# mathwrx/Decouple-and-Couple_Learning_in_Multi-Modal_Brain_Tumor_Segmentation

Hardware: AMD Instinct MI355X
Metric: training volumes/sec (4x128^3) (higher is better)
Workload: dtype bf16x3 forward (split-bf16 MFMA operands hi.hi+hi.lo+lo.hi: logits within 1e-3 of the fp32 reference) / bf16 data-gradient / bf16 weight-gradient MFMA operands; f32 accumulate, f32 storage, f32 master weights; 1 GPU; configs[1]: 1xMI355X, batch 2 per GPU, 4-modality 128^3 synthetic BraTS patches; fwd + softmax_dice + 4 sub-region/edge losses + bwd + Adam(amsgrad); random-init weights, dropout on; global_batch=2, parallelism=dp1, precision=bf16x3, dgrad_precision=bf16, wgrad_precision=bf16, mode=plan

## Files before the change

decouple-and-couple_learning_in_multi-modal_brain_tumor_segmentation_amd/csrc/wgrad_bf16.hip:

```cpp
#include "conv_args.h"
#include <type_traits>
#include <cstdlib>

typedef __bf16 bf16x8 __attribute__((ext_vector_type(8)));
typedef short s16x4 __attribute__((ext_vector_type(4)));
typedef __attribute__((address_space(3))) s16x4 lds_s16x4;

extern "C" int cwf_wgrad_nsplit(int op, int N, int Do, int Ho, int Wo, int Cin, int Cout);
constexpr int SIDE_WGS = 160;

struct WgArgsB {
  ConvGeom g;
  const float* x; const float* in_scale; const float* in_shift; float in_slope;
  const float* dy; int dy_ldc; float* partial;
  int ngroups, tiles_per_split, total_tiles;
  int64_t slab_floats;
  int cls_slab_base[8];
  int groups;
  const float* x_g[3]; const float* dy_g[3]; float* partial_g[3];
  const float* dy_scale;
};

__device__ __forceinline__ unsigned pack_bf16w(float a, float b) {
  const __bf16 x = (__bf16)a, y = (__bf16)b;
// ... 1031 lines not shown
#pragma unroll
    for (int i = 0; i < 7; ++i)
#pragma unroll
      for (int j = 0; j < NTW; ++j) acc[i][j] = (f32x4){0.f, 0.f, 0.f, 0.f};
    typedef short s16x8 __attribute__((ext_vector_type(8)));
    const s16x8 ones_s = {0x3F80, 0x3F80, 0x3F80, 0x3F80, 0x3F80, 0x3F80, 0x3F80, 0x3F80};
    const bf16x8 ones = __builtin_bit_cast(bf16x8, ones_s);
    const bool bias_wave = wave == 3;
    const unsigned lane_x = lds_base + (((kq & 1) * XW + (kq >> 1) * 8 + bq) * 16 + bp * 4) * 2;
    unsigned xa0[7];
#pragma unroll
    for (int i = 0; i < 7; ++i) {
      const int t = wave + 4 * i;
      xa0[i] = lane_x + (t < 27 ? (((t / 9) * 6 + (t / 3) % 3) * XW + t % 3) * 32 : 0);
    }
    const unsigned da0 = lds_base + WS1D_XIB + (((kq & 1) * DP + (kq >> 1) * 8 + bq) * CGW + (kq & 1) * DSK + bp * 4) * 2;
    auto trf = [&](unsigned addr, unsigned second) __attribute__((always_inline)) {
      const s16x4 u = __builtin_amdgcn_ds_read_tr16_b64_v4i16((lds_s16x4*)(uintptr_t)addr);
      const s16x4 v = __builtin_amdgcn_ds_read_tr16_b64_v4i16((lds_s16x4*)(uintptr_t)(addr + second));
      const s16x8 w = {u[0], u[1], u[2], u[3], v[0], v[1], v[2], v[3]};
      return __builtin_bit_cast(bf16x8, w);
    };
    for (int it = 0; it < niter; ++it) {
      asm volatile("s_barrier" ::: "memory");
      const unsigned bo = (unsigned)(it & 3) * WS1D_BUFB;
      unsigned xa[7];
#pragma unroll
      for (int i = 0; i < 7; ++i) xa[i] = xa0[i] + bo;
      const unsigned da = da0 + bo;
      constexpr int DEPTH = CWF_WS1_DEPTH;
      bf16x8 ah[DEPTH + 1], bh[2][NTW];
      auto issue = [&](int f) __attribute__((always_inline)) {
        const int ks = f / 7, i = f % 7;
        if (i == 0) {
          const unsigned od_ = (2 * ks * DP * CGW + ks * DSK) * 2;
#pragma unroll
          for (int j = 0; j < NTW; ++j) bh[ks & 1][j] = trf(da + od_ + j * 32, 4 * CGW * 2);
        }
        const unsigned ox = (((ks >> 1) * 6 + ((2 * ks) & 3)) * XW) * 32;
        ah[f % (DEPTH + 1)] = trf(xa[i] + ox, 4 * 32);
      };
#pragma unroll
      for (int f = 0; f < DEPTH; ++f) issue(f);
#pragma unroll
      for (int f = 0; f < 56; ++f) {
        if (f + DEPTH < 56) issue(f + DEPTH);
        __builtin_amdgcn_sched_barrier(0);
        const int ks = f / 7, i = f % 7;
        bf16x8 ahf = ah[f % (DEPTH + 1)];
        if (i == 6) ahf = bias_wave ? ones : ahf;
#pragma unroll
        for (int j = 0; j < NTW; ++j)
          acc[i][j] = __builtin_amdgcn_mfma_f32_16x16x32_bf16(ahf, bh[ks & 1][j], acc[i][j], 0, 0, 0);
        __builtin_amdgcn_sched_barrier(0);
      }
    }
    float4* out = reinterpret_cast<float4*>(a.partial + (int64_t)split * a.slab_floats);
#pragma unroll
    for (int i = 0; i < 7; ++i) {
      const int t = wave + 4 * i;
      if (t > 27) continue;
#pragma unroll
      for (int j = 0; j < NTW; ++j) {
        const int64_t blk = (((int64_t)chunk * a.ngroups + grp) * 28 + t) * CG + j;
        out[blk * 64 + lane] = make_float4(acc[i][j][0], acc[i][j][1], acc[i][j][2], acc[i][j][3]);
      }
    }
  } else {
    const int lw = wave - 4;
    typedef __attribute__((address_space(3))) void* lds_vp;
    typedef __attribute__((address_space(1))) const void* glb_vp;
    const int gx = a.Cin >> 3, gd = a.Cout >> 3;
    auto run = [&](auto NI_) __attribute__((always_inline)) {
      constexpr int NI = decltype(NI_)::value;
      int off[NI]; unsigned crd[NI];
#pragma unroll
      for (int k = 0; k < NI; ++k) {
        const int s = lw + WS1_LW * k;
        if (s < WS1D_XP) {
          const int gi = 64 * s + lane;
          const int row = gi / 40, gr = gi % 40, w = gr >> 1, half = gr & 1;
          const int c0 = row / 6, c1 = row % 6;
          off[k] = ((c0 * a.H + c1) * a.W + w) * gx + chunk * 2 + half;
          crd[k] = (unsigned)c0 | ((unsigned)c1 << 3) | ((unsigned)w << 6) | ((row < 36 && gr < 36) ? 1u << 11 : 0u);
        } else {
          const int m = s - WS1D_XP, w = lane >> 2, q = lane & 3;
          off[k] = (((m >> 2) * a.H + (m & 3)) * a.W + w) * gd + grp * 4 + q;
          crd[k] = (unsigned)(m >> 2) | ((unsigned)(m & 3) << 3) | ((unsigned)w << 6) | (1u << 11);
        }
      }
      auto issue = [&](int it) __attribute__((always_inline)) {
        const int tile = t_begin + it;
        const int n = tile / tiles_sp; int rem = tile - n * tiles_sp;
        const int tile_w = rem % a.tiles_w; rem /= a.tiles_w;
        const int tile_h = rem % a.tiles_h; const int tile_d = rem / a.tiles_h;
        const int od0 = tile_d * 4, oh0 = tile_h * 4, ow0 = tile_w * 16;
        const int64_t vd = (((int64_t)n * a.D + od0) * a.H + oh0) * a.W + ow0;
        const int64_t vx = vd - ((int64_t)a.H + 1) * a.W - 1;
        const unsigned lbuf = lds_base + (unsigned)(it & 3) * WS1D_BUFB;
#pragma unroll
        for (int k = 0; k < NI; ++k) {
          const int s = lw + WS1_LW * k;
          const bool isd = s >= WS1D_XP;
          const int c0 = (int)(crd[k] & 7u), c1 = (int)((crd[k] >> 3) & 7u), w = (int)((crd[k] >> 6) & 31u);
          const int gdd = (isd ? od0 : od0 - 1) + c0, gh = (isd ? oh0 : oh0 - 1) + c1, gw = (isd ? ow0 : ow0 - 1) + w;
          const bool ok = (crd[k] >> 11) != 0u && (unsigned)gdd < (unsigned)a.D && (unsigned)gh < (unsigned)a.H && (unsigned)gw < (unsigned)a.W;
          const uint4* src = (isd ? a.dy + vd * gd : a.xa + vx * gx) + off[k];
          src = ok ? src : a.zero;
          const int m = s - WS1D_XP;
          const unsigned dst = isd ? (unsigned)(WS1D_XIB + m * 1024 + ((m + 1) >> 1) * 32) : (unsigned)s * 1024u;
          __builtin_amdgcn_global_load_lds((glb_vp)src, (lds_vp)(uintptr_t)(lbuf + dst), 16, 0, 0);
        }
      };
      if (niter > 0) issue(0);
      if (niter > 1) issue(1);
      if (niter > 2) issue(2);
      for (int it = 0; it < niter; ++it) {
        if (it + 2 < niter) asm volatile("s_waitcnt vmcnt(%0)" :: "n"(2 * NI) : "memory");
        else asm volatile("s_waitcnt vmcnt(0)" ::: "memory");
        asm volatile("s_barrier" ::: "memory");
        if (it + 3 < niter) issue(it + 3);
      }
    };
    constexpr int NP = WS1D_XP + WS1D_DP;
    if (lw < NP % WS1_LW) run(std::integral_constant<int, NP / WS1_LW + 1>{});
    else run(std::integral_constant<int, NP / WS1_LW>{});
  }
}

static int wgrad_s1d_launch(const cwf_wgrad_args& d, int* nsplit_used, hipStream_t st) {
  const void* xa16 = d.xa16; const void* dy16 = d.dy16; const void* zero16 = d.zero16; float* partial = d.partial;
  const int N = d.N, D = d.Di, H = d.Hi, W = d.Wi, Cin = d.Cin, Cout = d.Cout;
  if (!xa16 || !dy16 || !zero16 || !partial || N <= 0 || D <= 0 || H <= 0 || W <= 0) return CWF_E_BADARG;
  if (((uintptr_t)xa16 & 15) || ((uintptr_t)dy16 & 15) || ((uintptr_t)zero16 & 15) || ((uintptr_t)partial & 15)) return CWF_E_ALIGN;
  if (Cin < 16 || (Cin & 15) || Cout < 32 || (Cout & 31)) return CWF_E_BADARG;
  if ((int64_t)N * D * H * W * (Cin > Cout ? Cin : Cout) >= (1ll << 33)) return CWF_E_TOOLARGE;
  Ws1dArgs a;
  a.xa = (const uint4*)xa16; a.dy = (const uint4*)dy16; a.zero = (const uint4*)zero16; a.partial = partial;
  a.N = N; a.D = D; a.H = H; a.W = W; a.Cin = Cin; a.Cout = Cout;
  a.tiles_d = cdiv(D, 4); a.tiles_h = cdiv(H, 4); a.tiles_w = cdiv(W, 16);
  a.total_tiles = N * a.tiles_d * a.tiles_h * a.tiles_w;
  const int nchunks = Cin / 16;
  a.ngroups = Cout / 32;
  const int nblk = nchunks * a.ngroups;
  a.slab_floats = (int64_t)nblk * 28 * 2 * 256;
  if (a.slab_floats != cwf_wgrad_slab_floats(CWF_CONV3_S1, Cin, Cout)) return CWF_E_BADARG;
  int want = SIDE_WGS / nblk; if (want < 1) want = 1; if (want > a.total_tiles) want = a.total_tiles;
  a.tiles_per_split = cdiv(a.total_tiles, want);
  const int splits = cdiv(a.total_tiles, a.tiles_per_split);
  if (splits > cwf_wgrad_nsplit(CWF_CONV3_S1, N, D, H, W, Cin, Cout)) return CWF_E_BADARG;
  const size_t lds = (size_t)WS1D_NBUF * WS1D_BUFB;
  CWF_MAX_LDS_ONCE((&wgrad_s1d_kernel));
  hipLaunchKernelGGL(wgrad_s1d_kernel, dim3(splits, nblk), dim3(256 + 64 * WS1_LW), lds, st, a);
  CWF_LAUNCH_CHECK();
  if (nsplit_used) *nsplit_used = splits;
  return 0;
}

struct PwWgWork { int Vin, gps, wps, gpw; };

template <int NCH, int NTL, int NCLS> struct PwgCfg { static constexpr int WAVES = (NCLS * NTL * (NCH + 1) <= 12) ? 16 : 8; };
template <int NCH, int NTL, int NCLS>
__global__ __launch_bounds__((64 * PwgCfg<NCH, NTL, NCLS>::WAVES)) void pw_wgrad_kernel(const WgArgsB a, const PwWgWork wk, int CG) {
  constexpr int PWG_WAVES = PwgCfg<NCH, NTL, NCLS>::WAVES, RB = 32 / PWG_WAVES;
  constexpr int G = (NCLS > 1) ? (NCH * NTL > 1 ? 1 : 2) : (NCH + NTL <= 2 ? 16 : (NCH + NTL <= 3 ? 12 : (NCH + NTL <= 6 ? 4 : 2)));
  __shared__ float4 red[PWG_WAVES][RB][64];
  const ConvGeom& g = a.g;
  const int tid = threadIdx.x, lane = tid & 63, li = lane & 15, lk = lane >> 4;
  const int wave = __builtin_amdgcn_readfirstlane(tid >> 6);
  const int n = (int)blockIdx.x / wk.wps, wg = (int)blockIdx.x % wk.wps;
  const int gA = (wg * PWG_WAVES + wave) * wk.gpw;
  const int gB = min(gA + wk.gpw, wk.gps);
  const float* xs = a.x + (int64_t)n * wk.Vin * g.x_ldc;
  const float* ds = a.dy + (int64_t)n * g.Do * g.Ho * g.Wo * a.dy_ldc;
  const bool has_norm = a.in_scale != nullptr;
  const bool plain = !has_norm && a.in_slope == 1.f;
  float sc[NCH], sh[NCH];
#pragma unroll
  for (int c = 0; c < NCH; ++c) {
    const int ci = c * 16 + li;
    sc[c] = (has_norm && ci < g.Cin) ? a.in_scale[(int64_t)n * g.Cin + ci] : 1.f;
    sh[c] = (has_norm && ci < g.Cin) ? a.in_shift[(int64_t)n * g.Cin + ci] : 0.f;
  }
  f32x4 acc[NCLS][NCH][NTL], accb[NCLS][NTL];
#pragma unroll
  for (int q = 0; q < NCLS; ++q)
#pragma unroll
    for (int t = 0; t < NTL; ++t) {
      accb[q][t] = (f32x4){0.f, 0.f, 0.f, 0.f};
#pragma unroll
      for (int c = 0; c < NCH; ++c) acc[q][c][t] = (f32x4){0.f, 0.f, 0.f, 0.f};
    }

  for (int gi = gA; gi < gB; gi += G) {
    float xv[G][NCH], dv[G][NCLS][NTL];
#pragma unroll
    for (int k = 0; k < G; ++k) {
      const bool ok = gi + k < gB;
      const int vox = (gi + k) * 4 + lk;
#pragma unroll
      for (int c = 0; c < NCH; ++c) {
        const int ci = c * 16 + li;
        xv[k][c] = (ok && ci < g.Cin) ? xs[(int64_t)vox * g.x_ldc + ci] : 0.f;
      }
      int64_t ov[NCLS];
      if (NCLS == 1) ov[0] = vox;
      else {
        const int w_ = vox % g.Wi, t2 = vox / g.Wi, h_ = t2 % g.Hi, d_ = t2 / g.Hi;
#pragma unroll
        for (int q = 0; q < NCLS; ++q) ov[q < NCLS ? q : 0] = ((int64_t)(2 * d_ + (q >> 2)) * g.Ho + 2 * h_ + ((q >> 1) & 1)) * g.Wo + 2 * w_ + (q & 1);
      }
#pragma unroll
      for (int q = 0; q < NCLS; ++q)
#pragma unroll
        for (int t = 0; t < NTL; ++t) {
          const int co = t * 16 + li;
          dv[k][q][t] = (ok && co < g.Cout) ? ds[ov[q] * a.dy_ldc + co] : 0.f;
        }
    }
#pragma unroll
    for (int k = 0; k < G; ++k) {
      const bool ok = gi + k < gB;
      float xa[NCH];
#pragma unroll
      for (int c = 0; c < NCH; ++c) {
        float v = xv[k][c];
        if (!plain) v = cwf_act(v * sc[c] + sh[c], a.in_slope);
        xa[c] = (ok && c * 16 + li < g.Cin) ? v : 0.f;
      }
#pragma unroll
      for (int q = 0; q < NCLS; ++q)
#pragma unroll
        for (int t = 0; t < NTL; ++t) {
          accb[q][t] = __builtin_amdgcn_mfma_f32_16x16x4f32(1.f, dv[k][q][t], accb[q][t], 0, 0, 0);
#pragma unroll
          for (int c = 0; c < NCH; ++c) acc[q][c][t] = __builtin_amdgcn_mfma_f32_16x16x4f32(xa[c], dv[k][q][t], acc[q][c][t], 0, 0, 0);
        }
    }
  }

  float4* out = reinterpret_cast<float4*>(a.partial + (int64_t)blockIdx.x * a.slab_floats);
  constexpr int NB = NCLS * NTL * (NCH + 1);
  f32x4 flat[NB]; int bid[NB];
  {
    int u = 0;
#pragma unroll
    for (int q = 0; q < NCLS; ++q)
#pragma unroll
      for (int t = 0; t < NTL; ++t) {
        const int grp = t / CG, j = t % CG;
#pragma unroll
        for (int c = 0; c < NCH; ++c) { flat[u] = acc[q][c][t]; bid[u] = a.cls_slab_base[q] + ((c * a.ngroups + grp) * 2) * CG + j; ++u; }
        flat[u] = accb[q][t]; bid[u] = a.cls_slab_base[q] + ((0 * a.ngroups + grp) * 2 + 1) * CG + j; ++u;
      }
  }
#pragma unroll
  for (int b0 = 0; b0 < NB; b0 += RB) {
    __syncthreads();
#pragma unroll
    for (int r_ = 0; r_ < RB; ++r_)
      if (b0 + r_ < NB) red[wave][r_][lane] = make_float4(flat[b0 + r_][0], flat[b0 + r_][1], flat[b0 + r_][2], flat[b0 + r_][3]);
    __syncthreads();
    if (wave < RB && b0 + wave < NB) {
      float4 sum = red[0][wave][lane];
#pragma unroll
      for (int w = 1; w < PWG_WAVES; ++w) { const float4 p = red[w][wave][lane]; sum.x += p.x; sum.y += p.y; sum.z += p.z; sum.w += p.w; }
      int id = bid[b0];
#pragma unroll
      for (int r_ = 1; r_ < RB; ++r_) if (b0 + r_ < NB && wave == r_) id = bid[b0 + r_];
      out[(int64_t)id * 64 + lane] = sum;
      if (NCH > 1) {
#pragma unroll
        for (int r_ = 0; r_ < RB; ++r_) {
          if (b0 + r_ < NB && wave == r_ && (b0 + r_) % (NCH + 1) == NCH) {
            for (int c = 1; c < NCH; ++c) out[((int64_t)id + (int64_t)c * a.ngroups * 2 * CG) * 64 + lane] = sum;
          }
        }
      }
    }
  }
}

template <int NCH, int NTL, int NCLS>
static int launch_pw_wgrad(const WgArgsB& a, int CG, int max_slabs, int* nsplit_used, hipStream_t st) {
  const ConvGeom& g = a.g;
  PwWgWork wk;
  wk.Vin = g.Di * g.Hi * g.Wi;
  wk.gps = wk.Vin >> 2;
  int wps = SIDE_WGS / g.N; if (wps < 1) wps = 1;
  if (wps * g.N > max_slabs) wps = max_slabs / g.N;
  if (wps < 1) return -1;
  constexpr int PWG_WAVES = PwgCfg<NCH, NTL, NCLS>::WAVES;
  const int maxw = cdiv(wk.gps, PWG_WAVES * 8);
  if (wps > maxw) wps = maxw;
  wk.gpw = cdiv(wk.gps, wps * PWG_WAVES);
  wk.wps = cdiv(wk.gps, wk.gpw * PWG_WAVES);
  hipLaunchKernelGGL((pw_wgrad_kernel<NCH, NTL, NCLS>), dim3((unsigned)(wk.wps * g.N)), dim3(64 * PWG_WAVES), 0, st, a, wk, CG);
  CWF_LAUNCH_CHECK();
  if (nsplit_used) *nsplit_used = wk.wps * g.N;
  return 0;
}

static int wgrad_bf16_impl(const cwf_wgrad_args& d, int* nsplit_used, hipStream_t st) {
  const int op = d.op, x3 = d.precision == CWF_BF16X3, groups = d.groups, N = d.N, Cin = d.Cin, Cout = d.Cout;
  const int Di = d.Di, Hi = d.Hi, Wi = d.Wi, Do = d.Do, Ho = d.Ho, Wo = d.Wo, x_ldc = d.x_ldc, dy_ldc = d.dy_ldc;
  const float* x = groups ? d.x_g[0] : d.x; const float* dy = groups ? d.dy_g[0] : d.dy; float* partial = groups ? d.partial_g[0] : d.partial;
  const float* in_scale = d.in_scale; const float* dy_scale = d.dy_scale;
  if (!x || !dy || !partial || N <= 0) return CWF_E_BADARG;
  if (dy_scale && !(!groups && op == CWF_CONV3_S1 && Cin <= 16 && Cout == 16 && (dy_ldc & 3) == 0 && (((uintptr_t)dy) & 15) == 0 && (int64_t)Do * Ho * Wo >= 32768))
    return CWF_E_BADARG;
  if ((Cin & 3) || (x_ldc & 3) || ((uintptr_t)x & 15) || ((uintptr_t)partial & 15)) return CWF_E_ALIGN;
  if (in_scale && !d.in_shift) return CWF_E_BADARG;
  if (!(op == CWF_CONV3_S1 || op == CWF_CONV3_S2 || op == CWF_CONV1 || op == CWF_CONVT2)) return CWF_E_BADARG;
  const bool tapsplit = (op == CWF_CONV3_S1 || op == CWF_CONV3_S2);
  const int MTOT = (op == CWF_CONV3_S2) ? 4 : 16;
  const int nt_all = cdiv(Cout, 16);
  const int CG = tapsplit ? (nt_all == 1 ? 1 : 2) : (nt_all == 1 ? 1 : (nt_all == 2 ? 2 : 4));
  WgArgsB a;
  int rc = cwf_build_geom(a.g, op, N, Di, Hi, Wi, Cin, x_ldc, Do, Ho, Wo, Cout, dy_ldc, MTOT);
  if (rc) return rc;
  const int nchunks = a.g.nchunks, ncls = a.g.ncls, ngroups = cdiv(a.g.ntiles, CG);
  int64_t blocks = 0;
  for (int c = 0; c < 8; ++c) { a.cls_slab_base[c] = (int)blocks; if (c < ncls) blocks += (int64_t)nchunks * ngroups * (a.g.cls_ntaps[c] + 1) * CG; }
  const int total = N * a.g.tiles_d * a.g.tiles_h * a.g.tiles_w;
  const int nblk = nchunks * ngroups * ncls;
  int want = 512 / nblk; if (want < 1) want = 1; if (want > total) want = total;
  const int tps = cdiv(total, want);
  const int wg_splits = cdiv(total, tps);
  if ((tapsplit ? wg_splits : wg_splits * 4) != cwf_wgrad_nsplit(op, N, Do, Ho, Wo, Cin, Cout) || blocks * 256 != cwf_wgrad_slab_floats(op, Cin, Cout))
    return CWF_E_BADARG;
  a.x = x; a.in_scale = in_scale; a.in_shift = d.in_shift; a.in_slope = d.in_slope; a.dy = dy; a.dy_ldc = dy_ldc; a.partial = partial;
  a.ngroups = ngroups; a.tiles_per_split = tps; a.total_tiles = total; a.slab_floats = blocks * 256;
  a.groups = groups; a.dy_scale = dy_scale;
  bool dy_al = (((uintptr_t)dy) & 15) == 0;
  for (int q = 0; q < 3; ++q) {
    a.x_g[q] = (groups && q < groups) ? d.x_g[q] : nullptr; a.dy_g[q] = (groups && q < groups) ? d.dy_g[q] : nullptr;
    a.partial_g[q] = (groups && q < groups) ? d.partial_g[q] : nullptr;
    if (groups && q < groups && (((uintptr_t)d.dy_g[q]) & 15)) dy_al = false;
  }
  const int gz = groups ? groups : ncls;
  if (nsplit_used) *nsplit_used = tapsplit ? wg_splits : wg_splits * 4;
  if (!groups && op == CWF_CONV3_S1 && Cin <= 16 && Cout == 16 && (dy_ldc & 3) == 0 && (((uintptr_t)dy) & 15) == 0 && (int64_t)Do * Ho * Wo >= 32768) {
    int grid = Cin <= 4 ? 256 : SIDE_WGS; while (grid > 8 && grid > total) grid -= 8;
    const size_t lds16 = (size_t)2 * (36 * W16_XW * 16 + 16 * W16_DW * 16) * sizeof(unsigned short) * (x3 ? 2 : 1);
    if (x3) {
      CWF_MAX_LDS_ONCE((&wgrad16_kernel<true>));
      hipLaunchKernelGGL((wgrad16_kernel<true>), dim3(grid), dim3(256 + 64 * W16_LW), lds16, st, a, total);
    } else {
      CWF_MAX_LDS_ONCE((&wgrad16_kernel<false>));
      hipLaunchKernelGGL((wgrad16_kernel<false>), dim3(grid), dim3(256 + 64 * W16_LW), lds16, st, a, total);
    }
    CWF_LAUNCH_CHECK();
    if (nsplit_used) *nsplit_used = grid;
    return 0;
  }
  if (!groups && (op == CWF_CONV1 || op == CWF_CONVT2) && ((int64_t)Di * Hi * Wi & 3) == 0 && (op == CWF_CONV1 || (Wi & 3) == 0) &&
      (int64_t)Di * Hi * Wi * (x_ldc > 8 * dy_ldc ? x_ldc : 8 * dy_ldc) < (1ll << 31)) {
    const int nch = nchunks, ntl = a.g.ntiles;
    const int max_slabs = wg_splits * 4;
    int r = -2;
    if (op == CWF_CONV1) {
      if (nch == 1 && ntl == 1) r = launch_pw_wgrad<1, 1, 1>(a, CG, max_slabs, nsplit_used, st);
      else if (nch == 2 && ntl == 1) r = launch_pw_wgrad<2, 1, 1>(a, CG, max_slabs, nsplit_used, st);
      else if (nch == 4 && ntl == 2) r = launch_pw_wgrad<4, 2, 1>(a, CG, max_slabs, nsplit_used, st);
      else if (nch == 8 && ntl == 4) r = launch_pw_wgrad<8, 4, 1>(a, CG, max_slabs, nsplit_used, st);
    } else {
      if (nch == 1 && ntl == 1) r = launch_pw_wgrad<1, 1, 8>(a, CG, max_slabs, nsplit_used, st);
      else if (nch == 2 && ntl == 2) r = launch_pw_wgrad<2, 2, 8>(a, CG, max_slabs, nsplit_used, st);
    }
    if (r >= 0) return r;
  }
  if (!x3 && op == CWF_CONV3_S1 && CG <= 2 && a.g.TD == 4 && a.g.TH == 4 && a.g.ID == 6 && a.g.IH == 6 && a.g.IW == 18 && (Cout & 3) == 0 &&
      (dy_ldc & 3) == 0 && dy_al) {
    int want1 = SIDE_WGS / nblk; if (want1 < 1) want1 = 1; if (want1 > total) want1 = total;
    const int tps1 = cdiv(total, want1), splits1 = cdiv(total, tps1);
    if (splits1 <= wg_splits) {
      a.tiles_per_split = tps1;
      if (nsplit_used) *nsplit_used = splits1;
      const size_t lds1 = (size_t)2 * (36 * 20 * 16 + 16 * (CG == 1 ? 20 : 16) * CG * 16 + (16 / 2 + 1) * (CG == 2 ? 16 : 0)) * sizeof(unsigned short);
      dim3 grid1(splits1, nchunks * ngroups, groups ? groups : 1);
      CWF_MAX_LDS_ONCE((&wgrad_s1_kernel<1>));
      CWF_MAX_LDS_ONCE((&wgrad_s1_kernel<2>));
      if (CG == 1) hipLaunchKernelGGL((wgrad_s1_kernel<1>), grid1, dim3(256 + 64 * WS1_LW), lds1, st, a);
      else hipLaunchKernelGGL((wgrad_s1_kernel<2>), grid1, dim3(256 + 64 * WS1_LW), lds1, st, a);
      CWF_LAUNCH_CHECK();
      return 0;
    }
  }
  const size_t ximg = (size_t)a.g.ID * a.g.IH * wg_x_pitch(a.g.IW, a.g.is) * 16;
  const size_t dimg = (size_t)a.g.TD * a.g.TH * wg_dy_pitch(CG * 16) * CG * 16 + (size_t)(a.g.TD * a.g.TH / 2 + 1) * wg_dy_skew(CG * 16);
  const size_t lds = (ximg + dimg) * sizeof(unsigned short) * (x3 ? 2 : 1);
  if (lds > 160 * 1024) return CWF_E_TOOLARGE;
  dim3 grid(wg_splits, nchunks * ngroups, gz);
#define CWF_WG(tpw, ntw, ts, xx) do { CWF_MAX_LDS_ONCE((&wgrad_bf16_kernel<tpw, ntw, ts, xx>)); \
    hipLaunchKernelGGL((wgrad_bf16_kernel<tpw, ntw, ts, xx>), grid, dim3(256), lds, st, a); } while (0)
#define CWF_WGX(tpw, ntw, ts) do { if (x3) CWF_WG(tpw, ntw, ts, true); else CWF_WG(tpw, ntw, ts, false); } while (0)
  if (tapsplit) { if (CG == 1) CWF_WGX(7, 1, true); else CWF_WGX(7, 2, true); }
  else { if (CG == 1) CWF_WGX(2, 1, false); else if (CG == 2) CWF_WGX(2, 2, false); else CWF_WGX(2, 4, false); }
#undef CWF_WGX
#undef CWF_WG
  CWF_LAUNCH_CHECK();
  return 0;
}

extern "C" int cwf_wgrad(const struct cwf_wgrad_args* args, int* nsplit_used, void* stream) {
  if (!args) return CWF_E_BADARG;
  const cwf_wgrad_args& d = *args;
  if (d.precision != CWF_FP32 && d.precision != CWF_BF16X3 && d.precision != CWF_BF16) return CWF_E_BADARG;
  hipStream_t st = cwf_stream(stream);
  if (d.xa16 || d.dy16) {
    if (!d.xa16 || !d.dy16 || d.precision != CWF_BF16 || d.op != CWF_CONV3_S1 || d.groups || d.dy_scale) return CWF_E_BADARG;
    if (d.Cin == 16 && d.Cout == 16 && (int64_t)d.Do * d.Ho * d.Wo >= 32768) return wgrad16_launch(d, nsplit_used, st);
    return wgrad_s1d_launch(d, nsplit_used, st);
  }
  if (d.groups) {
    if (d.groups < 2 || d.groups > 3 || d.op != CWF_CONV3_S1 || d.precision == CWF_FP32 || d.in_scale || d.dy_scale) return CWF_E_BADARG;
    for (int q = 0; q < d.groups; ++q)
      if (!d.x_g[q] || !d.dy_g[q] || !d.partial_g[q] || ((uintptr_t)d.x_g[q] & 15) || ((uintptr_t)d.partial_g[q] & 15)) return CWF_E_ALIGN;
    return wgrad_bf16_impl(d, nsplit_used, st);
  }
  if (d.precision == CWF_FP32) return d.dy_scale ? CWF_E_BADARG : wgrad_fp32_launch(d, nsplit_used, st);
  return wgrad_bf16_impl(d, nsplit_used, st);
}
```

decouple-and-couple_learning_in_multi-modal_brain_tumor_segmentation_amd/cwf/kernels.py:

```python
from __future__ import annotations

import ctypes

import threading

import numpy as np
import torch

from . import _lib
from . import packing as pk

_f32 = torch.float32


def cl(t: torch.Tensor):
    assert t.dim() == 5 and t.dtype == _f32, (t.shape, t.dtype)
    n, d, h, w, c = t.shape
    s = t.stride()
    ldc = s[3]
    ok = s[4] == 1 and ldc >= c and ldc % 4 == 0 and s[2] == w * ldc and s[1] == h * w * ldc and s[0] == d * h * w * ldc \
        and t.data_ptr() % 16 == 0
    if not ok:
        t = t.contiguous()
        ldc = c
# ... 53 lines not shown
    if which == "normal":
        return torch.cuda.Stream(device=device)
    if which == "high":
        return torch.cuda.Stream(device=device, priority=torch.cuda.Stream.priority_range()[1])
    import ctypes
    hip = ctypes.CDLL("libamdhip64.so")
    least, greatest = ctypes.c_int(0), ctypes.c_int(0)
    with torch.cuda.device(device):
        if hip.hipDeviceGetStreamPriorityRange(ctypes.byref(least), ctypes.byref(greatest)) != 0 or least.value <= 0:
            return torch.cuda.Stream(device=device, priority=torch.cuda.Stream.priority_range()[1])
        h = ctypes.c_void_p()
        if hip.hipStreamCreateWithPriority(ctypes.byref(h), ctypes.c_uint(1), ctypes.c_int(least.value)) != 0:
            raise RuntimeError("hipStreamCreateWithPriority failed")
    return torch.cuda.ExternalStream(h.value, device=device)


class HipBackend:
    name = "hip"

    def __init__(self):
        self.lib = _lib.load()
        if not torch.cuda.is_available():
            raise _lib.CwfError("no GPU visible: the cwf kernels are gfx950-only and there is no CPU fallback")
        self._ws = {}
        self._arena = {}
        self._arena_off = {}
        self._rng = {}
        self._rng_seed = {}
        self._site = 0
        self._wg_stream = {}
        self._wg_part = {}
        self._wg_pending = []
        self._wg_held = []
        self._wg_keep = []
        self.flush_every_default = 10
        self.flush_every = self.flush_every_default
        self.wgrad_defer = False
        self._wg_tables = {}
        self.wgrad_async = False
        self._rng_lock = threading.Lock()

    @staticmethod
    def _stream():
        return _raw_stream(_current_device())

    def _call(self, name, *args):
        rc = getattr(self.lib, name)(*args)
        if rc != 0:
            raise _lib.CwfError("%s failed with status %d" % (name, rc))

    def workspace(self, key, nfloats, device):
        k = (key, device, _raw_stream(_current_device()), torch.cuda.is_current_stream_capturing())
        buf = self._ws.get(k)
        if buf is None or buf.numel() < nfloats:
            buf = torch.empty(int(nfloats), dtype=_f32, device=device)
            self._ws[k] = buf
        return buf

    ARENA_DOUBLES = 1 << 20

    def rng(self, device):
        device = torch.device(device)
        st = self._rng.get(device)
        seed = torch.initial_seed() & 0x7FFFFFFFFFFFFFFF
        if st is None or (self._rng_seed.get(device) != seed and not torch.cuda.is_current_stream_capturing()):
            st = torch.tensor([seed, 0], dtype=torch.int64, device=device)
            self._rng[device] = st
            self._rng_seed[device] = seed
        return st

    def rng_site(self, n):
        with self._rng_lock:
            off = self._site
            self._site = off + 2 * int(n)
        return off

    def begin_step(self, device):
        self._call("cwf_rng_advance", self.rng(device).data_ptr(), self._stream())
        self._site = 0
        a = self._arena.get(device)
        if a is None:
            a = torch.zeros(self.ARENA_DOUBLES, dtype=torch.float64, device=device)
            self._arena[device] = a
        else:
            a.zero_()
        self._arena_off[device] = 0

    def _zeros_f64(self, shape, device):
        n = 1
        for s in shape:
            n *= s
        device = torch.device(device)
        a = self._arena.get(device)
        if a is not None:
            off = self._arena_off[device]
            if off + n <= a.numel():
                self._arena_off[device] = off + ((n + 1) // 2) * 2
                return a[off:off + n].view(shape)
        return torch.zeros(shape, dtype=torch.float64, device=device)

    def conv(self, op, x, wpk, bias, cout, in_scale=None, in_shift=None, slope=1.0, residual=None, out_scale=None,
             stats=None, out=None, w_ref=None, out_channels_alloc=None, fwd_op=None, prec=None, nb=None, bias_ref=None, x16=None, y16=None):
        x, x_ldc = cl(x)
        n, di, hi, wi, cin = x.shape
        if op == pk.CONV3_S2_DGRAD or op == pk.CONVT2_DGRAD:
            assert out is not None, "dgrad ops need an explicit output (its extent is not implied)"
        if out is None:
            do, ho, wo = pk.out_dims(op, di, hi, wi)
            ca = out_channels_alloc or cout
            out = torch.empty((n, do, ho, wo, ca), dtype=_f32, device=x.device)
        y = out
        _, do, ho, wo, _ = y.shape
        mode = prec or ((_DGRAD_PRECISION or _PRECISION) if (fwd_op is not None) else _PRECISION)
        a = _lib.ConvArgs(op=op, precision=_lib.PRECISION[mode], x=x.data_ptr(), x_ldc=x_ldc, wpk=wpk.data_ptr(), bias=_p(bias),
                          y=y.data_ptr(), y_ldc=y.stride(3), in_scale=_p(in_scale), in_shift=_p(in_shift), in_slope=float(slope),
                          out_scale=_p(out_scale), stats=_p(stats), nb_slope=1.0,
                          N=n, Di=di, Hi=hi, Wi=wi, Cin=cin, Do=do, Ho=ho, Wo=wo, Cout=cout)
        if residual is not None:
            residual, a.r_ldc = cl(residual)
            a.residual = residual.data_ptr()
        if nb is not None:
            nb_x, nb_scale, nb_shift, a.nb_slope = nb
            nb_x, a.nb_ldc = cl(nb_x)
            a.nb_x, a.nb_scale, a.nb_shift = nb_x.data_ptr(), nb_scale.data_ptr(), nb_shift.data_ptr()
        if x16 is not None:
            assert x16.dtype == torch.bfloat16 and x16.is_contiguous() and tuple(x16.shape) == (n, di, hi, wi, 16)
            a.x16, a.zero16 = x16.data_ptr(), self.zero16(x.device).data_ptr()
        if y16 is not None:
            assert y16.dtype == torch.bfloat16 and y16.is_contiguous()
            a.y16 = y16.data_ptr()
        if fwd_op is None and torch.is_tensor(w_ref) and w_ref.is_contiguous() and w_ref.dtype == _f32:
            a.w_raw = w_ref.data_ptr()
        self._call("cwf_conv", ctypes.addressof(a), self._stream())
        return y

    def supports_fused_norm_bwd(self, prec=None):
        return (prec or _PRECISION) != "fp32"

    def in_bwd_apply(self, dy, x, scale, shift, slope, sums, dx_add=None):
        dy, dy_ldc = cl(dy)
        x, x_ldc = cl(x)
        n, d, h, w, c = x.shape
        dx = torch.empty((n, d, h, w, c), dtype=_f32, device=x.device)
        a_ldc = 0
        if dx_add is not None:
            dx_add, a_ldc = cl(dx_add)
        self._call("cwf_in_bwd_apply", dy.data_ptr(), dy_ldc, x.data_ptr(), x_ldc, scale.data_ptr(), shift.data_ptr(), float(slope),
                   sums.data_ptr(), _p(dx_add), a_ldc, dx.data_ptr(), c, n, d * h * w, c, self._stream())
        return dx

    APPLY_EMITS = ("xa", "dx")

    def bf16_operands_ok(self, op, cin, cout, nvox):
        if op != pk.CONV3_S1 or (_WGRAD_PRECISION or _PRECISION) != "bf16":
            return 0
        if cin == 16 and cout == 16 and nvox >= 32768:
            return 16
        if cin >= 32 and cin % 16 == 0 and cout % 32 == 0:
            return 32
        return 0

    def bf16_dgrad_ok(self, op, cin, cout, nvox):
        return op == pk.CONV3_S1 and cin == 16 and cout == 16 and nvox >= 32768 and (_DGRAD_PRECISION or _PRECISION) == "bf16"

    def zero16(self, device):
        z = getattr(self, "_zero16", None)
        if z is None:
            z = self._zero16 = {}
        device = torch.device(device)
        t = z.get(device)
        if t is None:
            t = z[device] = torch.zeros(64, dtype=torch.uint8, device=device)
        return t

    def in_bwd_apply16(self, dy, x, scale, shift, slope, sums, dx_add=None, want_dx16=False, want_xa16=False, need_f32=True):
        dy, dy_ldc = cl(dy)
        x, x_ldc = cl(x)
        n, d, h, w, c = x.shape
        dx = torch.empty((n, d, h, w, c), dtype=_f32, device=x.device)
        if not need_f32 and POISON_UNWRITTEN_CARRIERS:
            dx.fill_(float("nan"))
        dx16 = torch.empty((n, d, h, w, c), dtype=torch.bfloat16, device=x.device) if want_dx16 else None
        xa16 = torch.empty((n, d, h, w, c), dtype=torch.bfloat16, device=x.device) if want_xa16 else None
        assert need_f32 or dx16 is not None
        a_ldc = 0
        if dx_add is not None:
            dx_add, a_ldc = cl(dx_add)
        self._call("cwf_in_bwd_apply_ex", dy.data_ptr(), dy_ldc, x.data_ptr(), x_ldc, scale.data_ptr(), shift.data_ptr(), float(slope),
                   sums.data_ptr(), _p(dx_add), a_ldc, dx.data_ptr() if need_f32 else 0, c, _p(dx16), _p(xa16), n, d * h * w, c, self._stream())
        return dx, dx16, xa16

    def to_bf16(self, x, scale=None, shift=None, slope=1.0, out=None):
        x, x_ldc = cl(x)
        n, d, h, w, c = x.shape
        y = out if out is not None else torch.empty((n, d, h, w, c), dtype=torch.bfloat16, device=x.device)
        assert y.dtype == torch.bfloat16 and y.is_contiguous() and tuple(y.shape) == (n, d, h, w, c)
        self._call("cwf_to_bf16", x.data_ptr(), x_ldc, _p(scale), _p(shift), float(slope), y.data_ptr(), n, d * h * w, c, self._stream())
        return y

    def to_bf16_side(self, x, scale, shift, slope):
        if not self.wgrad_async:
            return self.to_bf16(x, scale, shift, slope)
        side = self.wgrad_stream(x.device)
        side.wait_stream(torch.cuda.current_stream(x.device))
        with torch.cuda.stream(side):
            y = self.to_bf16(x, scale, shift, slope)
        for t in (x, scale, shift):
            if t is not None:
                t.record_stream(side)
        y.record_stream(torch.cuda.current_stream(x.device))
        return y

    def conv_grouped(self, x_all, cin, wpks, biases, cout, y_all, x_goff, y_goff, w_refs=None, fwd_op=None, prec=None):
        x_all, x_ldc = cl(x_all)
        y, y_ldc = cl(y_all)
        n, d, h, w, _ = x_all.shape
        G = len(wpks)
        mode = prec or ((_DGRAD_PRECISION or _PRECISION) if (fwd_op is not None) else _PRECISION)
        a = _lib.ConvArgs(op=pk.CONV3_S1, precision=_lib.PRECISION[mode], x=x_all.data_ptr(), x_ldc=x_ldc, y=y.data_ptr(), y_ldc=y_ldc,
                          in_slope=1.0, nb_slope=1.0, groups=G, x_goff=x_goff, y_goff=y_goff,
                          N=n, Di=d, Hi=h, Wi=w, Cin=cin, Do=d, Ho=h, Wo=w, Cout=cout)
        for q in range(G):
            a.wpk_g[q] = wpks[q].data_ptr()
            a.bias_g[q] = 0 if biases is None else _p(biases[q])
        self._call("cwf_conv", ctypes.addressof(a), self._stream())
        return y_all


    def wgrad_stream(self, device):
        st = self._wg_stream.get(device)
        if st is None:
            st = _priority_stream(device, "low")
            self._wg_stream[device] = st
        return st

    def join_wgrad_stream(self):
        for st in self._wg_stream.values():
            torch.cuda.current_stream(st.device).wait_stream(st)
        self._wg_keep.clear()

    def wgrad(self, op, x, in_scale, in_shift, slope, dy, cout, inv_map, has_bias_map, w_numel, w_ref_shape=None, prec=None, allow_async=False):
        if self.wgrad_async and allow_async:
            side = self.wgrad_stream(x.device)
            side.wait_stream(torch.cuda.current_stream(x.device))
            with torch.cuda.stream(side):
                out = self._wgrad_impl(op, x, in_scale, in_shift, slope, dy, cout, inv_map, has_bias_map, w_numel, w_ref_shape, prec)
            for t in (x, dy, in_scale, in_shift):
                if t is not None:
                    t.record_stream(side)
            return out
        return self._wgrad_impl(op, x, in_scale, in_shift, slope, dy, cout, inv_map, has_bias_map, w_numel, w_ref_shape, prec)

    def wgrad_release(self):
        self.wgrad_defer = False
        held, self._wg_held = self._wg_held, []
        if not held:
            return
        if not self.wgrad_async:
            for args in held:
                self.wgrad_to(*args, allow_async=True)
            return
        dev = held[0][2].device
        side = self.wgrad_stream(dev)
        side.wait_stream(torch.cuda.current_stream(dev))
        with torch.cuda.stream(side):
            for args in held:
                self._wgrad_to_impl(*args)
        self._wg_keep.extend(held)

    def channel_sum_to(self, dy, out, allow_async=False):
        if self.wgrad_async and allow_async:
            side = self.wgrad_stream(dy.device)
            side.wait_stream(torch.cuda.current_stream(dy.device))
            with torch.cuda.stream(side):
                self.stats_channel_sum(self.in_stats(dy), out)
            dy.record_stream(side)
        else:
            self.stats_channel_sum(self.in_stats(dy), out)
            self._wg_sync_needed = self.wgrad_async

    def dy_scale_ok(self, op, cin, cout, nvox):
        return op == pk.CONV3_S1 and cin <= 16 and cout == 16 and nvox >= 32768 and (_WGRAD_PRECISION or _PRECISION) != "fp32" and \
            not self.bf16_operands_ok(op, cin, cout, nvox)

    def wgrad_to(self, key, op, x, in_scale, in_shift, slope, dy, cout, inv_map, dw_dst, db_dst, prec=None, x16=None, dy16=None, dy_scale=None,
                 allow_async=False):
        if dy_scale is not None:
            self._check_dy_scale(op, x, dy, cout, prec, dy_scale)
        if self.wgrad_async and allow_async and self.wgrad_defer:
            self._wg_held.append((key, op, x, in_scale, in_shift, slope, dy, cout, inv_map, dw_dst, db_dst, prec, x16, dy16, dy_scale))
            return
        if self.wgrad_async and allow_async:
            side = self.wgrad_stream(x.device)
            side.wait_stream(torch.cuda.current_stream(x.device))
            with torch.cuda.stream(side):
                self._wgrad_to_impl(key, op, x, in_scale, in_shift, slope, dy, cout, inv_map, dw_dst, db_dst, prec, x16, dy16, dy_scale)
            for t in (x, dy, in_scale, in_shift, x16, dy16, dy_scale):
                if t is not None:
                    t.record_stream(side)
        else:
            self._wgrad_to_impl(key, op, x, in_scale, in_shift, slope, dy, cout, inv_map, dw_dst, db_dst, prec, x16, dy16, dy_scale)
            self._wg_sync_needed = self.wgrad_async
        if len(self._wg_pending) >= self.flush_every:
            self.wgrad_flush(x.device)

    def _check_dy_scale(self, op, x, dy, cout, prec, dy_scale):
        n, do, ho, wo = dy.shape[0], dy.shape[1], dy.shape[2], dy.shape[3]
# ... 1090 lines not shown
```

Baseline: 114.5 volumes/s.

## Add pre-packed bf16 weight-gradient kernel for stride-2 3x3x3 convolutions

Adds a dedicated stride-2 weight-gradient kernel that consumes bf16 activation and gradient operands already emitted by the preceding apply pass. Producer waves stream tiles into a 4-deep LDS ring with global_load_lds, and consumer waves do transposed LDS reads feeding 16x16x32 bf16 MFMAs. The host dispatch routes CONV3_S2 to the new path when channels align. The goal is to avoid the on-the-fly normalize, activate and convert work and the fp32 loads of the generic wgrad path for downsampling convs. In exchange it adds a new, complex kernel whose bounds and padding logic must be correct.

```diff
diff --git a/decouple-and-couple_learning_in_multi-modal_brain_tumor_segmentation_amd/csrc/wgrad_bf16.hip b/decouple-and-couple_learning_in_multi-modal_brain_tumor_segmentation_amd/csrc/wgrad_bf16.hip
--- a/decouple-and-couple_learning_in_multi-modal_brain_tumor_segmentation_amd/csrc/wgrad_bf16.hip
+++ b/decouple-and-couple_learning_in_multi-modal_brain_tumor_segmentation_amd/csrc/wgrad_bf16.hip
@@ -1207,6 +1207,197 @@
   const size_t lds = (size_t)WS1D_NBUF * WS1D_BUFB;
   CWF_MAX_LDS_ONCE((&wgrad_s1d_kernel));
   hipLaunchKernelGGL(wgrad_s1d_kernel, dim3(splits, nblk), dim3(256 + 64 * WS1_LW), lds, st, a);
+  CWF_LAUNCH_CHECK();
+  if (nsplit_used) *nsplit_used = splits;
+  return 0;
+}
+
+#define WS2D_XW 34
+#define WS2D_XP 27
+#define WS2D_DP 4
+#define WS2D_XIB (WS2D_XP * 1024)
+#define WS2D_DIB (4 * 1024 + 2 * 32)
+#define WS2D_BUFB (WS2D_XIB + WS2D_DIB)
+#define WS2D_NBUF 4
+struct Ws2dArgs {
+  const uint4* xa; const uint4* dy; const uint4* zero; float* partial;
+  int N, Di, Hi, Wi, Do, Ho, Wo, Cin, Cout, tiles_d, tiles_h, tiles_w, total_tiles, tiles_per_split, ngroups;
+  int64_t slab_floats;
+};
+
+__global__ __launch_bounds__(256 + 64 * WS1_LW) void wgrad_s2d_kernel(const Ws2dArgs a) {
+  constexpr int NTW = 2, CG = 2, CGW = 32, XW = WS2D_XW, DP = 16, DSK = 16;
+  extern __shared__ float4 lds4[];
+  const int tid = threadIdx.x, lane = tid & 63;
+  const int wave = __builtin_amdgcn_readfirstlane(tid >> 6);
+  const int split = blockIdx.x;
+  const int chunk = blockIdx.y / a.ngroups, grp = blockIdx.y % a.ngroups;
+  const int tiles_sp = a.tiles_d * a.tiles_h * a.tiles_w;
+  const int t_begin = split * a.tiles_per_split;
+  const int t_end = min(a.total_tiles, t_begin + a.tiles_per_split);
+  const int niter = max(t_end - t_begin, 0);
+  const unsigned lds_base = (unsigned)(uintptr_t)(__attribute__((address_space(3))) void*)lds4;
+
+  if (wave < 4) {
+    const int kq = lane >> 4, bq = (lane & 15) >> 2, bp = lane & 3;
+    f32x4 acc[7][NTW];
+#pragma unroll
+    for (int i = 0; i < 7; ++i)
+#pragma unroll
+      for (int j = 0; j < NTW; ++j) acc[i][j] = (f32x4){0.f, 0.f, 0.f, 0.f};
+    typedef short s16x8 __attribute__((ext_vector_type(8)));
+    const s16x8 ones_s = {0x3F80, 0x3F80, 0x3F80, 0x3F80, 0x3F80, 0x3F80, 0x3F80, 0x3F80};
+    const bf16x8 ones = __builtin_bit_cast(bf16x8, ones_s);
+    const bool bias_wave = wave == 3;
+    const unsigned lane_x = lds_base + (((kq & 1) * 2 * XW + (kq >> 1) * 8 + bq) * 16 + bp * 4) * 2;
+    unsigned xa0[7];
+#pragma unroll
+    for (int i = 0; i < 7; ++i) {
+      const int t = wave + 4 * i;
+      const int tw = t % 3, col = tw == 0 ? 0 : (tw == 1 ? 17 : 1);
+      xa0[i] = lane_x + (t < 27 ? (((t / 9) * 5 + (t / 3) % 3) * XW + col) * 32 : 0);
+    }
+    const unsigned da0 = lds_base + WS2D_XIB + (((kq & 1) * DP + (kq >> 1) * 8 + bq) * CGW + (kq & 1) * DSK + bp * 4) * 2;
+    auto trf = [&](unsigned addr, unsigned second) __attribute__((always_inline)) {
+      const s16x4 u = __builtin_amdgcn_ds_read_tr16_b64_v4i16((lds_s16x4*)(uintptr_t)addr);
+      const s16x4 v = __builtin_amdgcn_ds_read_tr16_b64_v4i16((lds_s16x4*)(uintptr_t)(addr + second));
+      const s16x8 w = {u[0], u[1], u[2], u[3], v[0], v[1], v[2], v[3]};
+      return __builtin_bit_cast(bf16x8, w);
+    };
+    for (int it = 0; it < niter; ++it) {
+      asm volatile("s_barrier" ::: "memory");
+      const unsigned bo = (unsigned)(it & 3) * WS2D_BUFB;
+      unsigned xa[7];
+#pragma unroll
+      for (int i = 0; i < 7; ++i) xa[i] = xa0[i] + bo;
+      const unsigned da = da0 + bo;
+      constexpr int DEPTH = CWF_WS1_DEPTH;
+      bf16x8 ah[DEPTH + 1], bh[2][NTW];
+      auto issue = [&](int f) __attribute__((always_inline)) {
+        const int ks = f / 7, i = f % 7;
+        if (i == 0) {
+          const unsigned od_ = (2 * ks * DP * CGW + ks * DSK) * 2;
+#pragma unroll
+          for (int j = 0; j < NTW; ++j) bh[ks & 1][j] = trf(da + od_ + j * 32, 4 * CGW * 2);
+        }
+        ah[f % (DEPTH + 1)] = trf(xa[i] + ks * (2 * 5 * XW) * 32, 4 * 32);
+      };
+#pragma unroll
+      for (int f = 0; f < DEPTH; ++f) issue(f);
+#pragma unroll
+      for (int f = 0; f < 14; ++f) {
+        if (f + DEPTH < 14) issue(f + DEPTH);
+        __builtin_amdgcn_sched_barrier(0);
+        const int ks = f / 7, i = f % 7;
+        bf16x8 ahf = ah[f % (DEPTH + 1)];
+        if (i == 6) ahf = bias_wave ? ones : ahf;
+#pragma unroll
+        for (int j = 0; j < NTW; ++j)
+          acc[i][j] = __builtin_amdgcn_mfma_f32_16x16x32_bf16(ahf, bh[ks & 1][j], acc[i][j], 0, 0, 0);
+        __builtin_amdgcn_sched_barrier(0);
+      }
+    }
+    float4* out = reinterpret_cast<float4*>(a.partial + (int64_t)split * a.slab_floats);
+#pragma unroll
+    for (int i = 0; i < 7; ++i) {
+      const int t = wave + 4 * i;
+      if (t > 27) continue;
+#pragma unroll
+      for (int j = 0; j < NTW; ++j) {
+        const int64_t blk = (((int64_t)chunk * a.ngroups + grp) * 28 + t) * CG + j;
+        out[blk * 64 + lane] = make_float4(acc[i][j][0], acc[i][j][1], acc[i][j][2], acc[i][j][3]);
+      }
+    }
+  } else {
+    const int lw = wave - 4;
+    typedef __attribute__((address_space(3))) void* lds_vp;
+    typedef __attribute__((address_space(1))) const void* glb_vp;
+    const int gx = a.Cin >> 3, gd = a.Cout >> 3;
+    auto run = [&](auto NI_) __attribute__((always_inline)) {
+      constexpr int NI = decltype(NI_)::value;
+      int off[NI]; unsigned crd[NI];
+#pragma unroll
+      for (int k = 0; k < NI; ++k) {
+        const int s = lw + WS1_LW * k;
+        if (s < WS2D_XP) {
+          const int gi = 64 * s + lane;
+          const int row = gi / (2 * XW), gr = gi % (2 * XW), v = gr >> 1, half = gr & 1;
+          const int c0 = row / 5, c1 = row % 5;
+          const int w = v < 17 ? 2 * v : 2 * (v - 17) + 1;
+          off[k] = ((c0 * a.Hi + c1) * a.Wi + w) * gx + chunk * 2 + half;
+          crd[k] = (unsigned)c0 | ((unsigned)c1 << 3) | ((unsigned)w << 6) | ((row < 25 && v < 33) ? 1u << 12 : 0u);
+        } else {
+          const int m = s - WS2D_XP, w = lane >> 2, q = lane & 3;
+          off[k] = (((m >> 1) * a.Ho + (m & 1)) * a.Wo + w) * gd + grp * 4 + q;
+          crd[k] = (unsigned)(m >> 1) | ((unsigned)(m & 1) << 3) | ((unsigned)w << 6) | (1u << 12);
+        }
+      }
+      auto issue = [&](int it) __attribute__((always_inline)) {
+        const int tile = t_begin + it;
+        const int n = tile / tiles_sp; int rem = tile - n * tiles_sp;
+        const int tile_w = rem % a.tiles_w; rem /= a.tiles_w;
+        const int tile_h = rem % a.tiles_h; const int tile_d = rem / a.tiles_h;
+        const int od0 = tile_d * 2, oh0 = tile_h * 2, ow0 = tile_w * 16;
+        const int id0 = 2 * od0 - 1, ih0 = 2 * oh0 - 1, iw0 = 2 * ow0 - 1;
+        const int64_t vd = (((int64_t)n * a.Do + od0) * a.Ho + oh0) * a.Wo + ow0;
+        const int64_t vx = (((int64_t)n * a.Di + id0) * a.Hi + ih0) * a.Wi + iw0;
+        const unsigned lbuf = lds_base + (unsigned)(it & 3) * WS2D_BUFB;
+#pragma unroll
+        for (int k = 0; k < NI; ++k) {
+          const int s = lw + WS1_LW * k;
+          const bool isd = s >= WS2D_XP;
+          const int c0 = (int)(crd[k] & 7u), c1 = (int)((crd[k] >> 3) & 7u), w = (int)((crd[k] >> 6) & 63u);
+          const int gdd = (isd ? od0 : id0) + c0, gh = (isd ? oh0 : ih0) + c1, gw = (isd ? ow0 : iw0) + w;
+          const bool ok = (crd[k] >> 12) != 0u && (unsigned)gdd < (unsigned)(isd ? a.Do : a.Di) && (unsigned)gh < (unsigned)(isd ? a.Ho : a.Hi) &&
+                          (unsigned)gw < (unsigned)(isd ? a.Wo : a.Wi);
+          const uint4* src = (isd ? a.dy + vd * gd : a.xa + vx * gx) + off[k];
+          src = ok ? src : a.zero;
+          const int m = s - WS2D_XP;
+          const unsigned dst = isd ? (unsigned)(WS2D_XIB + m * 1024 + ((m + 1) >> 1) * 32) : (unsigned)s * 1024u;
+          __builtin_amdgcn_global_load_lds((glb_vp)src, (lds_vp)(uintptr_t)(lbuf + dst), 16, 0, 0);
+        }
+      };
+      if (niter > 0) issue(0);
+      if (niter > 1) issue(1);
+      if (niter > 2) issue(2);
+      for (int it = 0; it < niter; ++it) {
+        if (it + 2 < niter) asm volatile("s_waitcnt vmcnt(%0)" :: "n"(2 * NI) : "memory");
+        else asm volatile("s_waitcnt vmcnt(0)" ::: "memory");
+        asm volatile("s_barrier" ::: "memory");
+        if (it + 3 < niter) issue(it + 3);
+      }
+    };
+    constexpr int NP = WS2D_XP + WS2D_DP;
+    if (lw < NP % WS1_LW) run(std::integral_constant<int, NP / WS1_LW + 1>{});
+    else run(std::integral_constant<int, NP / WS1_LW>{});
+  }
+}
+
+static int wgrad_s2d_launch(const cwf_wgrad_args& d, int* nsplit_used, hipStream_t st) {
+  const void* xa16 = d.xa16; const void* dy16 = d.dy16; const void* zero16 = d.zero16; float* partial = d.partial;
+  const int N = d.N, Cin = d.Cin, Cout = d.Cout;
+  if (!xa16 || !dy16 || !zero16 || !partial || N <= 0 || d.Di <= 0 || d.Hi <= 0 || d.Wi <= 0) return CWF_E_BADARG;
+  if (d.Do != (d.Di - 1) / 2 + 1 || d.Ho != (d.Hi - 1) / 2 + 1 || d.Wo != (d.Wi - 1) / 2 + 1) return CWF_E_BADARG;
+  if (((uintptr_t)xa16 & 15) || ((uintptr_t)dy16 & 15) || ((uintptr_t)zero16 & 15) || ((uintptr_t)partial & 15)) return CWF_E_ALIGN;
+  if (Cin < 16 || (Cin & 15) || Cout < 32 || (Cout & 31)) return CWF_E_BADARG;
+  if ((int64_t)N * d.Di * d.Hi * d.Wi * (Cin > Cout ? Cin : Cout) >= (1ll << 33)) return CWF_E_TOOLARGE;
+  Ws2dArgs a;
+  a.xa = (const uint4*)xa16; a.dy = (const uint4*)dy16; a.zero = (const uint4*)zero16; a.partial = partial;
+  a.N = N; a.Di = d.Di; a.Hi = d.Hi; a.Wi = d.Wi; a.Do = d.Do; a.Ho = d.Ho; a.Wo = d.Wo; a.Cin = Cin; a.Cout = Cout;
+  a.tiles_d = cdiv(d.Do, 2); a.tiles_h = cdiv(d.Ho, 2); a.tiles_w = cdiv(d.Wo, 16);
+  a.total_tiles = N * a.tiles_d * a.tiles_h * a.tiles_w;
+  const int nchunks = Cin / 16;
+  a.ngroups = Cout / 32;
+  const int nblk = nchunks * a.ngroups;
+  a.slab_floats = (int64_t)nblk * 28 * 2 * 256;
+  if (a.slab_floats != cwf_wgrad_slab_floats(CWF_CONV3_S2, Cin, Cout)) return CWF_E_BADARG;
+  int want = SIDE_WGS / nblk; if (want < 1) want = 1; if (want > a.total_tiles) want = a.total_tiles;
+  a.tiles_per_split = cdiv(a.total_tiles, want);
+  const int splits = cdiv(a.total_tiles, a.tiles_per_split);
+  if (splits > cwf_wgrad_nsplit(CWF_CONV3_S2, N, d.Do, d.Ho, d.Wo, Cin, Cout)) return CWF_E_BADARG;
+  const size_t lds = (size_t)WS2D_NBUF * WS2D_BUFB;
+  CWF_MAX_LDS_ONCE((&wgrad_s2d_kernel));
+  hipLaunchKernelGGL(wgrad_s2d_kernel, dim3(splits, nblk), dim3(256 + 64 * WS1_LW), lds, st, a);
   CWF_LAUNCH_CHECK();
   if (nsplit_used) *nsplit_used = splits;
   return 0;
@@ -1464,7 +1655,9 @@
   if (d.precision != CWF_FP32 && d.precision != CWF_BF16X3 && d.precision != CWF_BF16) return CWF_E_BADARG;
   hipStream_t st = cwf_stream(stream);
   if (d.xa16 || d.dy16) {
-    if (!d.xa16 || !d.dy16 || d.precision != CWF_BF16 || d.op != CWF_CONV3_S1 || d.groups || d.dy_scale) return CWF_E_BADARG;
+    if (!d.xa16 || !d.dy16 || d.precision != CWF_BF16 || d.groups || d.dy_scale) return CWF_E_BADARG;
+    if (d.op == CWF_CONV3_S2) return wgrad_s2d_launch(d, nsplit_used, st);
+    if (d.op != CWF_CONV3_S1) return CWF_E_BADARG;
     if (d.Cin == 16 && d.Cout == 16 && (int64_t)d.Do * d.Ho * d.Wo >= 32768) return wgrad16_launch(d, nsplit_used, st);
     return wgrad_s1d_launch(d, nsplit_used, st);
   }
diff --git a/decouple-and-couple_learning_in_multi-modal_brain_tumor_segmentation_amd/cwf/kernels.py b/decouple-and-couple_learning_in_multi-modal_brain_tumor_segmentation_amd/cwf/kernels.py
--- a/decouple-and-couple_learning_in_multi-modal_brain_tumor_segmentation_amd/cwf/kernels.py
+++ b/decouple-and-couple_learning_in_multi-modal_brain_tumor_segmentation_amd/cwf/kernels.py
@@ -229,7 +229,11 @@
     APPLY_EMITS = ("xa", "dx")
 
     def bf16_operands_ok(self, op, cin, cout, nvox):
-        if op != pk.CONV3_S1 or (_WGRAD_PRECISION or _PRECISION) != "bf16":
+        if (_WGRAD_PRECISION or _PRECISION) != "bf16":
+            return 0
+        if op == pk.CONV3_S2:
+            return 32 if (cin % 16 == 0 and cout % 32 == 0) else 0
+        if op != pk.CONV3_S1:
             return 0
         if cin == 16 and cout == 16 and nvox >= 32768:
             return 16
```

Result: no change. 115.3 volumes/s (median of 6 runs) (+0.6%).
